# benjjneb/dada2

Measured on AMD Instinct MI355X. Metric: unique reads denoised/sec (dada() wall-clock), higher is better.
Workload: dtype int32 DP + f64 lambda/p-value

## Files before the change

dada2_amd/csrc/driver.cpp:

```cpp
#include <fcntl.h>
#include <sys/file.h>
#include <unistd.h>

#include <algorithm>
#include <atomic>
#include <chrono>
#include <condition_variable>
#include <deque>
#include <exception>
#include <mutex>
#include <cmath>
#include <cstdarg>
#include <cstdio>
#include <cstring>
#include <ctime>
#include <memory>
#include <thread>
#include <unordered_map>

#include "engine.h"
#include "hostpar.h"
#include "knobs.h"
#include "ppois.h"

// ... 45 lines not shown
  }
};

}

using namespace d2;

struct dada2hip_sample {
  int device = 0;
  hipStream_t stream = nullptr;
  hipStream_t side = nullptr;
  hipStream_t cmp = nullptr;
  SampleDev D;
  DevBuf<uint32_t> seq2, heavy, reads;
  DevBuf<uint8_t> qual, nheavy, prior;
  DevBuf<uint16_t> kord, kmult;
  DevBuf<uint32_t> kbits;
  DevBuf<int32_t> len, nwflag;
  PinBuf<uint32_t> h_seq2;
  std::vector<int32_t> h_len;
  std::vector<uint32_t> h_reads;
  std::vector<uint8_t> h_prior;
  uint64_t total_reads = 0;
  int qmax = 0;
  double ms_upload = 0;
  DevBuf<uint8_t> d_skip, d_cls, d_correct, d_moves;
  DevBuf<double> d_lambda, d_err;
  DevBuf<uint32_t> d_ham, scr_ptr, scr_t, d_qn, d_ctab, scr_adw, scr_ad;
  DevBuf<uint16_t> scr_foff;
  DevBuf<AdDesc> scr_fdesc;
  int scr_adw_waves = 0, scr_adw_band = -999;
// ... 241 lines not shown
  D2_HIP(hipMemcpyAsync(D.seq2, packed, (size_t)nraw * D.W2 * 4, hipMemcpyHostToDevice, s->stream));
  D2_HIP(hipMemcpyAsync(D.len, s->h_len.data(), (size_t)nraw * 4, hipMemcpyHostToDevice, s->stream));
  D2_HIP(hipMemcpyAsync(D.reads, s->h_reads.data(), (size_t)nraw * 4, hipMemcpyHostToDevice, s->stream));
  D2_HIP(hipMemcpyAsync(D.prior, s->h_prior.data(), (size_t)nraw, hipMemcpyHostToDevice, s->stream));
  if (lite) {
    D2_HIP(hipMemsetAsync(D.qual, 0, (size_t)nraw * D.LQ, s->stream));
    D2_HIP(hipStreamSynchronize(s->stream));
    s->qmax = 0;
    s->ms_upload = ms_since(t0);
    return;
  }
  s->kord.alloc((size_t)nraw * D.LK);
  s->heavy.alloc((size_t)nraw * std::max(D.HMAX, 1));
  D.kord = s->kord.p; D.heavy = s->heavy.p;
  if (maxlen - KMER_SIZE + 1 <= 512 && knobs().screen_bits != 0) {
    s->kbits.alloc((size_t)nraw * 32); s->kmult.alloc(nraw);
    D.kbits = s->kbits.p; D.kmult = s->kmult.p;
  } else { D.kbits = nullptr; D.kmult = nullptr; }
  launch_build_kmers(D, s->stream);

  {
    const int LQ = D.LQ;
    PinBuf<uint8_t> hq;
    hq.alloc((size_t)nraw * LQ);
    std::atomic<int> badq{0}, qmax{0};
    const int marshal_threads = active_runs(device).load() > 1 ? std::max(8, HostPool::get().nthreads() / 2) : 0;
    const size_t rows_per = std::max<size_t>(1, ((size_t)16 << 20) / (size_t)LQ);
    for (size_t r0 = 0; r0 < (size_t)nraw; r0 += rows_per) {
      const size_t nr = std::min<size_t>(rows_per, nraw - r0);
      parallel_for(nr, 512, [&](size_t lo, size_t hi) {
        int mx = 0, bad = 0;
        for (size_t r = r0 + lo; r < r0 + hi; r++) {
          const double *src = quals + r * (size_t)maxlen;
// ... 917 lines not shown
  PinBuf<Round2Out> v2_hblk;
  DevBuf<unsigned long long> v2_trace;
  int v2_trace_seq = -1;
  int v2_nbuf = 64, v2_depth = 2, v2_chain = SH_CHAIN;
  bool v2_debug = false;
  bool v3_on = false;
  int v3_depth = 1;
  int v3_grid = 1;
  int v3_bs = 1024;
  long v3_enq = 0;
  long v3_ord_seen = 0;
  DevBuf<PSync> v3_psync;
  DevBuf<int32_t> v3_lockbuf;
  int v3_lock_stride = 0;
  bool v3_pf_lowreg = false;
  bool v3_overlap = false;
  Eng2 E2P{};
  SampleDev S2{};
  DevBuf<Ctl2> v3_pfctl;
  DevBuf<PfSync> v3_pfsync;
  DevBuf<uint2> v3_pf_tab8;
  DevBuf<uint16_t> v3_pf_full, v3_pf_ord, v3_pf_foff;
  DevBuf<int32_t> v3_pf_blist, v3_pf_blistn, v3_pf_bretry, v3_pf_bretryn;
  DevBuf<uint32_t> v3_pf_ad;
  DevBuf<AdDesc> v3_pf_fdesc;
  long v3_pf_launched = 0;
  long v3_pf_seen = 0;
  long v3_pf_chains = 0;
  bool v3_pf_gate_on = true;
  hipEvent_t v3_pf_ev[4] = {nullptr, nullptr, nullptr, nullptr};
// ... 153 lines not shown

    v3_grid = tail_grid(N, s->device);
    if (K.v3_grid > 0) v3_grid = std::min(K.v3_grid, tail_grid(1 << 30, s->device));
    v3_overlap = v3_on && !v2_align_commit && v2_nbuf >= 4 && K.v3_overlap != 0 && N >= 2 && (active_runs(s->device).load() <= 1 || K.v3_overlap == 1);
    v3_bs = K.v3_block == 512 ? 512 : 1024;
    {
      const int ncu = tail_grid(1 << 30, s->device);
      if (v3_overlap && K.v3_block == 0 && K.v3_grid == 0 && v3_grid > ncu / 2) {
        v3_bs = 1024;
        v3_grid = std::max(1, std::min((N + 8191) / 8192, ncu / 2));
      }
    }
    if (v3_on) { const int cap = tail_resident_max(s->device, v3_bs); if (cap == 0 || (cap > 0 && v3_grid > cap)) v3_on = false; }
    if (!v3_on) v3_overlap = false;
    v3_pf_lowreg = K.v3_pf_lowreg >= 0 ? K.v3_pf_lowreg != 0 : (v3_overlap && v3_bs == 512);
    v3_lock_stride = 0;
    if (v3_on) {
      const long long per_group = 4096ll * v3_grid;
      v3_lock_stride = (int)(((long long)N + per_group - 1) / per_group * 4096ll);
      v3_lockbuf.alloc((size_t)v3_lock_stride * (size_t)v3_grid);
    }
    v3_pf_launched = 0; v3_pf_seen = 0; v3_pf_chains = 0;
    if (v3_overlap) {
      if (!s->cmp) D2_HIP(hipStreamCreateWithFlags(&s->cmp, hipStreamNonBlocking));
      for (auto &e : v3_pf_ev) if (!e) D2_HIP(hipEventCreateWithFlags(&e, hipEventDisableTiming));
      const size_t npad = ((size_t)N + 31) & ~(size_t)15;
      v3_pfctl.alloc(1); v3_pfsync.alloc(1); v3_pf_tab8.alloc(NKMER); v3_pf_cbits.alloc(KB_MAX * 32); v3_pf_full.alloc((size_t)KB_MAX * NKMER);
      v3_pf_ord.alloc((size_t)KB_MAX * s->D.LK + 64); v3_pf_blist.alloc((size_t)2 * KB_MAX * npad); v3_pf_blistn.alloc(2 * KB_MAX);
      v3_pf_bretry.alloc((size_t)KB_MAX * npad); v3_pf_bretryn.alloc(KB_MAX);
      D2_HIP(hipMemsetAsync(v3_pf_bretryn.p, 0, KB_MAX * 4, stq));
// ... 52 lines not shown
    st.tail_fallbacks++;
    v2_enq = v2_cons;
    v2_enqrec.assign((size_t)v2_cons, EnqRec{-1, -1, false});
    v2_next_full = 0;
    if (knobs().v2_summary) fprintf(stderr, "[v3] entry barrier failed after %ld blocks: continuing on the launch chains\n", v2_cons);
  }
  bool v3_block_ready() const { return *(volatile int32_t *)&v2_hblk.p[v2_cons % RING2].seq == (int32_t)(v2_cons + 1); }
  long v3_ended() const { return (long)*(volatile int32_t *)(v3_hflags.p + 16); }
  std::vector<EnqRec> v3_rec;
  void v3_enqueue(bool first) {
    const auto t_enq = clk::now();
    hipStream_t stq = s->stream;
    EnqRec rec{-1, -1, !first};
    if (!first) {
      rec.ev_screen = ev_begin(EV_SCREEN, profile_all, true);
      launch2_screen_multi(E2, stq);
      ev_end(rec.ev_screen);
      launch2_batch_lists(E2, stq);
      const NwBatch nb{&v2_ctl.p->nalign, v2_blistn.p, v2_blist.p, v2_ctl.p->acentre, &v2_ctl.p->abuf, E2.C.Npad, v2_bretry.p, v2_bretryn.p, v2_retrytot.p, &v2_ctl.p->fast_off};
      launch_gapless_batch(s->D, nb, ap, s->d_err.p, v2_lamB.p, v2_hamB.p, &v2_ctl.p->state, stq);
      rec.ev_nw = ev_begin(EV_NW, profile_all, true);
      launch_nw_ad(s->D, -1, nullptr, nullptr, nullptr, 0, nullptr, nullptr, ap, s->d_err.p, v2_lamB.p, v2_hamB.p, nullptr, 0, 0, nullptr, stq,
                   &v2_ctl.p->state, &nb);
      ev_end(rec.ev_nw);
    }
    const int ev = ev_begin(EV_TAIL, profile_all);
    Eng2 Ek = E2;
    if (!profile_all) Ek.ktime = nullptr;
    Ek.pf_plan = (v3_overlap && (active_runs(s->device).load() <= 1 || knobs().v3_overlap == 1)) ? 1 : 0;
    launch3_tail(Ek, v3_grid, v3_bs, first, (int)(v3_enq + 1), s->h_reads[bi[0].center], stq);
    ev_end(ev);
    v3_rec.push_back(rec);
    v3_enq++;
    st.ms_enqueue += ms_since(t_enq);
  }

  void v3_pf_enqueue(long k) {
    const auto t_enq = clk::now();
    hipStream_t st2 = s->cmp;
    Ctl2 *pc = v3_pfctl.p;
    *(volatile int32_t *)(v3_hflags.p + 40 + (k & 7)) = 0;
    launch2_pf_gate(E2P, (int)k, v3_hflags.p + 32, v3_hflags.p + 40 + (k & 7), st2);
    launch2_pf_tables(E2P, st2);
    int ev = ev_begin(EV_PF_SCREEN, profile_all, false, false, st2);
    launch2_screen_multi(E2P, st2, v3_pf_lowreg);
    ev_end(ev);
    launch2_batch_lists(E2P, st2);
    const NwBatch nb{&pc->nalign, v3_pf_blistn.p, v3_pf_blist.p, pc->acentre, &pc->abuf, E2.C.Npad, v3_pf_bretry.p, v3_pf_bretryn.p, v2_retrytot.p, &pc->fast_off};
    launch_gapless_batch(S2, nb, ap, s->d_err.p, v2_lamB.p, v2_hamB.p, &pc->state, st2);
    ev = ev_begin(EV_PF_NW, profile_all, false, false, st2);
    launch_nw_ad(S2, -1, nullptr, nullptr, nullptr, 0, nullptr, nullptr, ap, s->d_err.p, v2_lamB.p, v2_hamB.p, nullptr, 0, 0, nullptr, st2,
                 &pc->state, &nb);
    ev_end(ev);
    launch2_pf_done(E2P, st2);
    D2_HIP(hipEventRecord(v3_pf_ev[k & 3], st2));
    v3_pf_launched = std::max(v3_pf_launched, k);
    v3_pf_chains++;
    st.ms_enqueue += ms_since(t_enq);
  }
  int v3_pf_gate_result(long k) const { return (int)*(volatile int32_t *)(v3_hflags.p + 40 + (k & 7)); }
// ... 308 lines not shown
    else {
      v2_round_launches(nlev, with_compare, store, &rec, lite);
      if (with_compare) v2_plain_rounds++;
    }
    if (lite) st.lite_chains++;
    v2_enqrec.push_back(rec);
    v2_enq++;
    st.ms_enqueue += ms_since(t_enq);
  }
  void v2_round_launches(int nlev, bool with_compare, bool store, EnqRec *recp, bool lite = false) {
    hipStream_t stq = s->stream;
    EnqRec rec{-1, -1, with_compare};
    const Eng2 &E2 = lite ? this->E2L : this->E2;
    if (with_compare && !lite) {
      rec.ev_screen = ev_begin(EV_SCREEN, profile_all, true);
      launch2_screen_multi(E2, stq);
      ev_end(rec.ev_screen);
      launch2_batch_lists(E2, stq);
      const NwBatch nb{&v2_ctl.p->nalign, v2_blistn.p, v2_blist.p, v2_ctl.p->acentre, &v2_ctl.p->abuf, E2.C.Npad, v2_bretry.p, v2_bretryn.p, v2_retrytot.p, &v2_ctl.p->fast_off};
      launch_gapless_batch(s->D, nb, ap, s->d_err.p, v2_lamB.p, v2_hamB.p, &v2_ctl.p->state, stq);
      rec.ev_nw = ev_begin(EV_NW, profile_all, true);
      launch_nw_ad(s->D, -1, nullptr, nullptr, nullptr, 0, nullptr, nullptr, ap, s->d_err.p, v2_lamB.p, v2_hamB.p, nullptr, 0, 0, nullptr, stq,
                   &v2_ctl.p->state, &nb);
      ev_end(rec.ev_nw);
    }
    int ev = ev_begin(EV_SHUFFLE, profile_all && nlev > 0);
    for (int l = 0; l < nlev; l++) launch2_shuffle(E2, l, store && l == 0, stq);
    ev_end(ev);
    ev = ev_begin(EV_PVAL, profile_all);
    launch2_eval(E2, nlev, s->h_reads[bi[0].center], stq);
    ev_end(ev);
// ... 1293 lines not shown
```

dada2_amd/csrc/engine.h:

```cpp
#pragma once
#include <cstddef>
#include <cstdint>
#include <string>
#include <vector>

#include <hip/hip_runtime.h>

#include "../../include/dada2hip.h"

namespace d2 {

constexpr int KMER_SIZE = 5;
constexpr int NKMER = 1024;
constexpr int RANK_SAT = 63;
constexpr int MAX_SHUFFLE = 10;
constexpr int SEQLEN = 9999;
constexpr double TAIL_APPROX_CUTOFF = 1e-7;

enum : uint8_t { CLS_SKIP = 0, CLS_SHROUD = 1, CLS_GAPLESS = 2, CLS_NW = 3 };

struct DeviceError {
  int code;
  std::string msg;
};
// ... 7 lines not shown
  } while (0)

struct SampleDev {
  int32_t N = 0, maxlen = 0, minlen = 0;
  int32_t r_lo = 0, r_hi = 0;
  int32_t W2 = 0;
  int32_t LQ = 0;
  int32_t LK = 0;
  int32_t HMAX = 0;
  uint32_t *seq2 = nullptr;
  uint8_t *qual = nullptr;
  uint16_t *kord = nullptr;
  uint32_t *heavy = nullptr;
  uint8_t *nheavy = nullptr;
  uint32_t *kbits = nullptr;
  uint16_t *kmult = nullptr;
  int32_t *len = nullptr;
  uint32_t *reads = nullptr;
  uint8_t *prior = nullptr;
  int32_t *nw_flag = nullptr;
  uint32_t *ad_ptr = nullptr;
  int32_t ad_waves = 0;
  int32_t ad_wpw = 0;
  uint16_t *ad_foff = nullptr;
  struct AdDesc *ad_desc = nullptr;
  int32_t ad_fcap = 0, ad_fstride = 0;
};

struct AdDesc { long long dest; int32_t L2, pad; };

struct AlignParams {
// ... 312 lines not shown
};

struct PSync {
  uint32_t arrive, pad0[31];
  uint32_t gen, pad1[31];
  uint32_t fail, pad2[31];
  uint32_t top, pad3[31];
  uint32_t ngrp, pad4[31];
  uint32_t xarr[8][32], xgen[8][32], xcount[8][32], xn[8][32];
};
enum { KT_S0 = 0, KT_S0_BAR, KT_SL, KT_SL_BAR, KT_P, KT_P_BAR, KT_BIRTH, KT_PUBLISH, KT_ROUNDS, KT_LEVELS, KT_LAUNCH, KT_RELEASE,
       KT_PFWAIT , KT_PLAN , KT_SUB_LAST = 14, KT_SUB = 16, KT_N = 80 };

void launch2_store0(const Eng2 &E, const double *d_lam, const uint32_t *d_ham, const uint8_t *d_cls, const int32_t *d_round_counters,
                    hipStream_t st);
void launch2_screen_multi(const Eng2 &E, hipStream_t st, bool beside_tail = false);
void launch2_pf_gate(const Eng2 &E, int k, const int32_t *h_quit, int32_t *h_result, hipStream_t st);
void launch2_pf_tables(const Eng2 &E, hipStream_t st);
void launch2_pf_done(const Eng2 &E, hipStream_t st);
void launch2_batch_lists(const Eng2 &E, hipStream_t st);
void launch2_shuffle(const Eng2 &E, int level, bool store, hipStream_t st);
void launch2_eval(const Eng2 &E, int nlev, uint32_t init_reads, hipStream_t st);
void launch2_host_birth(const Eng2 &E, int raw, int from, hipStream_t st);
void launch2_resume(const Eng2 &E, hipStream_t st, bool keep_list = false, bool compare_done = false);
void launch2_posthoc(const Eng2 &E, const int32_t *d_cluster_of_centre, int32_t *d_out_ji, double *d_out_lam, int32_t *d_nout,
                     int cap, hipStream_t st);
int tail_grid(int N, int device);
int tail_resident_max(int device, int bs);
int tail_mirror_cap(int device, int bs);
void launch3_tail(const Eng2 &E, int grid, int bs, bool first, int ordinal, uint32_t init_reads, hipStream_t st);

// ... 13 lines not shown
```

dada2_amd/csrc/kernels.hip:

```cpp
#include <cstring>

#include "engine.h"
#include "gcn.h"
#include "knobs.h"
#include "rounds_common.h"
#include "ppois.h"

namespace d2 {

static __device__ __forceinline__ uint32_t base_at(const uint32_t *__restrict__ row, int p) {
  return (row[p >> 4] >> ((p & 15) << 1)) & 3u;
}

static __device__ __forceinline__ uint32_t homo_at(const uint32_t *__restrict__ row, int len, int p) {
  if (p < 0 || p >= len) return 0u;
  const uint32_t b = base_at(row, p);
  const int l = (p >= 1 && base_at(row, p - 1) == b) ? ((p >= 2 && base_at(row, p - 2) == b) ? 2 : 1) : 0;
  const int r = (p + 1 < len && base_at(row, p + 1) == b) ? ((p + 2 < len && base_at(row, p + 2) == b) ? 2 : 1) : 0;
  return (l + r >= 2) ? 1u : 0u;
}

__global__ __launch_bounds__(64) void k_build_kmers(SampleDev S) {
  __shared__ uint16_t tbl[NKMER * 64];
  const int lane = threadIdx.x;
// ... 16 lines not shown
      }
      for (int i = nk; i < S.LK; i++) ko[i] = 0xFFFFu;
      int nh = 0;
      if (S.HMAX > 0 || S.kbits) {
        int distinct = 0;
        for (int w = 0; w < NKMER / 32; w++) {
          uint32_t bits = 0;
          for (int b = 0; b < 32; b++) {
            const int k = 32 * w + b;
            const uint32_t c = t[k * 64];
            if (c) { bits |= 1u << b; distinct++; }
            if (S.HMAX > 0 && c > RANK_SAT) S.heavy[(size_t)r * S.HMAX + nh++] = (uint32_t)k | (c << 16);
          }
          if (S.kbits) S.kbits[(size_t)r * 32 + w] = bits;
        }
        if (S.kmult) S.kmult[r] = (uint16_t)min(max(nk, 0) - distinct, 65535);
      }
      S.nheavy[r] = (uint8_t)nh;
    }
  }
}

void launch_build_kmers(const SampleDev &S, hipStream_t st) {
  int grid = std::min((S.N + 63) / 64, 1024);
  hipLaunchKernelGGL(k_build_kmers, dim3(grid), dim3(64), 0, st, S);
}

constexpr int CTAB_SAT = 0, CTAB_CNT = 256, CTAB_ORD = 768;
static __device__ __forceinline__ void centre_table_body(const SampleDev &S, int centre, uint32_t *__restrict__ ctab, uint32_t *cnt) {
  const int tid = threadIdx.x;
  for (int k = tid; k < NKMER; k += 256) cnt[k] = 0;
// ... 2450 lines not shown
```

dada2_amd/csrc/rounds2.inc.hip:

```cpp

#ifndef D2_PUPD_INLINE
#define D2_PUPD_INLINE __forceinline__
#endif
#ifndef D2_SHUF_INLINE
#define D2_SHUF_INLINE __forceinline__
#endif
#define D2_TRACE2(KID, SUBKID, PHASE)                                                                              \
  do {                                                                                                             \
    if (E.trace && threadIdx.x == 0 && (int)blockIdx.x < TRACE_BLOCKS && E.ctl->pub_seq == E.trace_seq)           \
      E.trace[((size_t)(KID) * TRACE_BLOCKS + blockIdx.x) * 8 + (PHASE)] = gcn_clock();                            \
    D2_KSUB(SUBKID, PHASE, blockIdx.x == 0);                                                                       \
  } while (0)
#define D2_TRACE(KID, PHASE) D2_TRACE2(KID, KID, PHASE)
#define D2_TRACE_SH(LEVEL, PHASE) D2_TRACE2(1 + (LEVEL), (LEVEL) == 0 ? 1 : 2, PHASE)
#ifdef D2_TAIL_TU
static __shared__ unsigned long long s_ktime[KT_N];
#define D2_KT s_ktime
#else
#define D2_KT E.ktime
#endif
#define D2_KSUB(KID, PHASE, WHO)                                                                                   \
  do {                                                                                                             \
    if (E.ktime && threadIdx.x == 0 && (WHO)) {                                                                    \
      const unsigned long long now_ = gcn_wall_clock();                                                            \
// ... 1402 lines not shown
  build_batch_tables(E.S, E.C, nb, E.ctl->bcentre, s_cnt);
}
__global__ void k2_pf_done(Eng2 E) {
  if (threadIdx.x != 0 || E.ctl->state != 0) return;
  unsigned long long nn = 0, ng = 0;
  for (int k = 0; k < KB_MAX; k++) { nn += (unsigned long long)E.blist_n[k]; ng += (unsigned long long)E.blist_n[KB_MAX + k]; }
  E.pfsync->nnw += nn; E.pfsync->ngapless += ng;
  gcn_release_agent();
  gcn_store_agent(&E.pfsync->done, (uint32_t)E.ctl->pf_seq);
}

struct ScrIn { uint4 c0, c1; int Lr, nh; uint32_t rd; bool lk; };

template <int WAVES>
__global__ __launch_bounds__(256, WAVES) void k2_screen_multi(Eng2 E) {
  const Ctl2 *ctl = E.ctl;
  const int nb = ctl->nbatch;
  if (ctl->state != 0 || nb == 0) return;
  extern __shared__ __attribute__((aligned(16))) uint32_t s_mem[];
  const SampleDev &S = E.S;
  const Cache2 &C = E.C;
  const ScreenParams sp = E.sp;
  uint2 *tab = (uint2 *)s_mem;
  uint16_t *cord = (uint16_t *)(tab + NKMER);
  int32_t *thr = (int32_t *)(cord + (size_t)KB_MAX * S.LK);
  __shared__ int cL[KB_MAX], cC[KB_MAX];
  __shared__ uint32_t cR[KB_MAX];
  const int tid = threadIdx.x;
  for (int i = tid; i < NKMER; i += 256) tab[i] = C.tab8[i];
  {
    const int n16 = (nb * S.LK * 2 + 15) / 16;
    const uint4 *src = (const uint4 *)C.ord;
    for (int i = tid; i < n16; i += 256) ((uint4 *)cord)[i] = src[i];
  }
  for (int i = tid; i < S.maxlen + 2; i += 256) thr[i] = E.thresh[i];
  if (tid < KB_MAX) { cL[tid] = ctl->blen[tid]; cC[tid] = ctl->bcentre[tid]; cR[tid] = ctl->breads[tid]; }
  __syncthreads();
  uint16_t *bcls = C.bcls + (size_t)ctl->bbuf * C.Npad;
  const int lane = tid & 63, sub = tid & 15, g = lane >> 4;
  const int gwave = blockIdx.x * 4 + (tid >> 6), nwaves = gridDim.x * 4;
  const int nchunk = (S.maxlen - KMER_SIZE + 1 + 7) >> 3;
  const uint4 pad4 = make_uint4(0xFFFFFFFFu, 0xFFFFFFFFu, 0xFFFFFFFFu, 0xFFFFFFFFu);
  const bool heavy_on = sp.use_kmers && S.HMAX > 0;
  const int kc = sub & 7;
  const bool kvalid = sub < 8 && kc < nb;
  const int Lc = cL[kc], Cc = cC[kc];
  const uint32_t Rc = cR[kc];
  auto load = [&](int r) __attribute__((always_inline)) {
    ScrIn in;
// ... 19 lines not shown
#pragma unroll
        for (int e = 0; e < 4; e++) {
#pragma unroll
          for (int hlf = 0; hlf < 2; hlf++) {
            const uint32_t x = hlf ? (w[e] >> 16) : (w[e] & 0xFFFFu);
            const uint2 t = tab[x & 1023u];
            const uint32_t rk = x >> 10;
            const uint32_t rr = gcn_bcast_byte0(rk);
            ax += ((t.x - rr) >> 7) & 0x01010101u;
            ay += ((t.y - rr) >> 7) & 0x01010101u;
          }
        }
        w0 += ax & 0x00FF00FFu; w1 += (ax >> 8) & 0x00FF00FFu;
        w2 += ay & 0x00FF00FFu; w3 += (ay >> 8) & 0x00FF00FFu;
      }
#pragma unroll
      for (int o = 8; o >= 1; o >>= 1) {
        w0 += __shfl_xor(w0, o, 16); w1 += __shfl_xor(w1, o, 16);
        w2 += __shfl_xor(w2, o, 16); w3 += __shfl_xor(w3, o, 16);
      }
    }
    uint32_t dot = (((kc & 4) ? ((kc & 1) ? w3 : w2) : ((kc & 1) ? w1 : w0)) >> ((kc & 2) ? 16 : 0)) & 0xFFFFu;
    const bool skipped = E.greedy && (in.rd > Rc || (in.lk && r != Cc));
    if (in.nh > 0 && kvalid && !skipped) {
      for (int hh = 0; hh < in.nh; hh++) {
        const uint32_t e = S.heavy[(size_t)r * S.HMAX + hh], cr = e >> 16, cc = C.full[(size_t)kc * NKMER + (e & 1023u)];
        const uint32_t m = cr < cc ? cr : cc;
        if (m > RANK_SAT) dot += m - RANK_SAT;
      }
      dot &= 0xFFFFu;
    }
    const int d = (Lc < in.Lr ? Lc : in.Lr) - KMER_SIZE + 1;
    const bool shroud = sp.use_kmers && (int)dot < thr[d > 0 ? d : 0];
    const bool gl_ok = sp.gapless && sp.use_kmers && (sp.sse >= 1 || in.Lr == Lc);
    bool gapless = sp.band == 0;
// ... 6 lines not shown
      const uint32_t dotk = (uint32_t)__shfl((int)dot, kk, 16);
      const uint16_t *ck = cord + (size_t)kk * S.LK;
      uint32_t ord = 0;
      for (int ch = sub, j = 0; ch < nchunk; ch += 16, j++) {
        const uint4 v = j == 0 ? in.c0 : (j == 1 ? in.c1 : row[ch]);
        const uint4 ck4 = ((const uint4 *)ck)[ch];
        const uint32_t w[4] = {v.x, v.y, v.z, v.w}, cw[4] = {ck4.x, ck4.y, ck4.z, ck4.w};
        const int i0 = ch << 3;
#pragma unroll
        for (int e = 0; e < 4; e++) {
          const uint32_t t = (w[e] ^ cw[e]) & 0x03FF03FFu;
          ord += ((t & 0xFFFFu) == 0 && i0 + 2 * e < dk);
          ord += ((t >> 16) == 0 && i0 + 2 * e + 1 < dk);
        }
      }
#pragma unroll
      for (int o = 8; o >= 1; o >>= 1) ord += __shfl_xor(ord, o, 16);
      if (kc == kk && sub < 8) gapless = (ord & 0xFFFFu) == dotk;
    }
    uint32_t c = !kvalid ? 0u : (skipped ? (uint32_t)CLS_SKIP : (shroud ? (uint32_t)CLS_SHROUD : (gapless ? (uint32_t)CLS_GAPLESS : (uint32_t)CLS_NW)));
    uint32_t code = c << (2 * kc);
    code |= __shfl_xor(code, 1, 16); code |= __shfl_xor(code, 2, 16); code |= __shfl_xor(code, 4, 16);
    return code & 0xFFFFu;
  };
  const bool pre = sp.use_kmers && S.kbits != nullptr && S.kmult != nullptr && C.cbits != nullptr;
  if (!pre) {
    for (int base16 = gwave * 16; base16 < S.N; base16 += nwaves * 16) {
      const int r0 = base16 + 4 * g;
      const ScrIn i0 = load(r0), i1 = load(r0 + 1);
      unsigned long long clsacc = one(r0, i0);
      const ScrIn i2 = load(r0 + 2);
      clsacc |= (unsigned long long)one(r0 + 1, i1) << 16;
      const ScrIn i3 = load(r0 + 3);
      clsacc |= (unsigned long long)one(r0 + 2, i2) << 32;
      clsacc |= (unsigned long long)one(r0 + 3, i3) << 48;
      if (sub == 0 && r0 < S.N) *(unsigned long long *)(bcls + r0) = clsacc;
    }
    return;
  }
  constexpr int SCR_ITERS = 8, SCR_LIST = SCR_ITERS * 64;
  __shared__ int s_list[SCR_LIST];
  __shared__ int s_nlist;
  __shared__ uint2 s_cbits[KB_MAX][16];
  if (tid < KB_MAX * 16) s_cbits[tid >> 4][tid & 15] = ((const uint2 *)C.cbits)[tid];
  if (tid == 0) s_nlist = 0;
  __syncthreads();
  const int wv = tid >> 6, grp = tid >> 4;
  auto flush = [&]() __attribute__((always_inline)) {
    __syncthreads();
    const int n = s_nlist;
    for (int q = grp; q < ((n + 15) & ~15); q += 32) {
      const bool ha = q < n, hb = q + 16 < n;
      const int ra = ha ? s_list[q] : s_list[0], rb = hb ? s_list[q + 16] : s_list[0];
      const ScrIn ia = load(ra), ib = load(rb);
      const uint32_t ca = one(ra, ia), cb = one(rb, ib);
      if (sub == 0 && ha) bcls[ra] = (uint16_t)ca;
      if (sub == 0 && hb) bcls[rb] = (uint16_t)cb;
    }
    __syncthreads();
    if (tid == 0) { if (n && E.fast_ctl) atomicAdd(&E.fast_ctl[3], (unsigned long long)n); s_nlist = 0; }
    __syncthreads();
  };
  int iter = 0;
  for (long long bb = (long long)blockIdx.x * 64; bb < S.N; bb += (long long)gridDim.x * 64, iter++) {
    const int r0 = (int)bb + 16 * wv + 4 * g;
    uint2 bw[4];
    int Ls[4], kms[4];
    uint32_t rds[4];
    bool lks[4];
#pragma unroll
    for (int u = 0; u < 4; u++) {
      const int r = r0 + u;
      const bool on = r < S.N;
      bw[u] = on ? ((const uint2 *)(S.kbits + (size_t)r * 32))[sub] : make_uint2(0u, 0u);
      Ls[u] = on ? S.len[r] : 0;
      rds[u] = on ? S.reads[r] : 0u;
      lks[u] = on && E.greedy && E.P.lock[r];
      kms[u] = on ? (int)S.kmult[r] : 0;
    }
    unsigned long long clsacc = 0;
    uint32_t survs = 0;
#pragma unroll
    for (int u = 0; u < 4; u++) {
      const int r = r0 + u;
      uint32_t p[4];
#pragma unroll
      for (int kk = 0; kk < 4; kk++) {
        const uint2 c0 = s_cbits[2 * kk][sub], c1 = s_cbits[2 * kk + 1][sub];
        const uint32_t n0 = (uint32_t)__popc(bw[u].x & c0.x) + (uint32_t)__popc(bw[u].y & c0.y);
        const uint32_t n1 = (uint32_t)__popc(bw[u].x & c1.x) + (uint32_t)__popc(bw[u].y & c1.y);
        p[kk] = n0 | (n1 << 16);
      }
#pragma unroll
      for (int o = 8; o >= 1; o >>= 1) {
        p[0] += __shfl_xor(p[0], o, 16); p[1] += __shfl_xor(p[1], o, 16);
        p[2] += __shfl_xor(p[2], o, 16); p[3] += __shfl_xor(p[3], o, 16);
      }
      const uint32_t pk = (kc & 4) ? ((kc & 2) ? p[3] : p[2]) : ((kc & 2) ? p[1] : p[0]);
      const int bound = (int)((pk >> ((kc & 1) ? 16 : 0)) & 0xFFFFu) + kms[u];
      const int d = (Lc < Ls[u] ? Lc : Ls[u]) - KMER_SIZE + 1;
      const bool skipped = E.greedy && (rds[u] > Rc || (lks[u] && r != Cc));
      const bool open = kvalid && r < S.N && !skipped && !(bound < thr[d > 0 ? d : 0]);
      uint32_t code = (kvalid ? (skipped ? (uint32_t)CLS_SKIP : (uint32_t)CLS_SHROUD) : 0u) << (2 * kc);
      code |= __shfl_xor(code, 1, 16); code |= __shfl_xor(code, 2, 16); code |= __shfl_xor(code, 4, 16);
      const bool any_open = ((__ballot(open) >> (16 * g)) & 0xFFFFull) != 0ull;
      if (any_open) survs |= 1u << u;
      clsacc |= (unsigned long long)(code & 0xFFFFu) << (16 * u);
    }
    if (sub == 0 && r0 < S.N) {
      if (survs == 0) *(unsigned long long *)(bcls + r0) = clsacc;
      else {
        int at = atomicAdd(&s_nlist, __popc(survs));
#pragma unroll
        for (int u = 0; u < 4; u++) {
          if (r0 + u >= S.N) continue;
          if ((survs >> u) & 1u) s_list[at++] = r0 + u;
          else bcls[r0 + u] = (uint16_t)(clsacc >> (16 * u));
        }
      }
    }
    if ((iter % SCR_ITERS) == SCR_ITERS - 1) flush();
  }
  flush();
}

__global__ __launch_bounds__(256) void k2_posthoc(Eng2 E, const int32_t *__restrict__ cluster_of_centre, int32_t *__restrict__ out_ji,
                                                  double *__restrict__ out_lam, int32_t *__restrict__ nout, int cap) {
  const int r = blockIdx.x * blockDim.x + threadIdx.x;
  if (r >= E.S.N) return;
  const int j = cluster_of_centre[r];
  if (j < 0) return;
  if (j != 0) {
    const int k = atomicAdd(nout, 1);
    if (k < cap) { out_ji[2 * k] = j; out_ji[2 * k + 1] = 0; out_lam[k] = E.T.lam0[r]; }
  }
  const int i1 = E.T.i1[r];
  if (i1 >= 0 && i1 != j) {
    const int k = atomicAdd(nout, 1);
// ... 12 lines not shown

void launch2_store0(const Eng2 &E, const double *d_lam, const uint32_t *d_ham, const uint8_t *d_cls, const int32_t *d_round_counters,
                    hipStream_t st) {
  const int grid = std::min((E.S.N + 255) / 256, 2048);
  hipLaunchKernelGGL(k2_store0, dim3(grid), dim3(256), 0, st, E, d_lam, d_ham, d_cls, d_round_counters);
}
void launch2_batch_lists(const Eng2 &E, hipStream_t st) {
  const int grid = (E.S.N + 256 * LISTS_PER_THREAD - 1) / (256 * LISTS_PER_THREAD);
  hipLaunchKernelGGL(k2_batch_lists, dim3(grid), dim3(256), 0, st, E);
}
void launch2_pf_gate(const Eng2 &E, int k, const int32_t *h_quit, int32_t *h_result, hipStream_t st) {
  hipLaunchKernelGGL(k2_pf_gate, dim3(1), dim3(64), 0, st, E, k, h_quit, h_result);
}
void launch2_pf_tables(const Eng2 &E, hipStream_t st) { hipLaunchKernelGGL(k2_pf_tables, dim3(1), dim3(1024), 0, st, E); }
void launch2_pf_done(const Eng2 &E, hipStream_t st) { hipLaunchKernelGGL(k2_pf_done, dim3(1), dim3(64), 0, st, E); }
void launch2_screen_multi(const Eng2 &E, hipStream_t st, bool beside_tail) {
  const size_t lds = (size_t)NKMER * 8 + (size_t)KB_MAX * E.S.LK * 2 + (size_t)(E.S.maxlen + 2) * 4 + 16;
  static size_t attr_set[64] = {0};
  int dev_ = 0;
  (void)hipGetDevice(&dev_);
  if (lds > attr_set[dev_ & 63]) {
    (void)hipFuncSetAttribute((const void *)k2_screen_multi<4>, hipFuncAttributeMaxDynamicSharedMemorySize, (int)lds);
    (void)hipFuncSetAttribute((const void *)k2_screen_multi<6>, hipFuncAttributeMaxDynamicSharedMemorySize, (int)lds);
    attr_set[dev_ & 63] = lds;
  }
  const int grid = std::min((E.S.N + 63) / 64, 2048);
  if (beside_tail) hipLaunchKernelGGL(k2_screen_multi<6>, dim3(grid), dim3(256), lds, st, E);
  else hipLaunchKernelGGL(k2_screen_multi<4>, dim3(grid), dim3(256), lds, st, E);
}
void launch2_shuffle(const Eng2 &E, int level, bool store, hipStream_t st) {
  const int grid = std::min((E.S.N + 255) / 256, (int)E.grid_shuffle);
  if (store) hipLaunchKernelGGL(k2_shuffle<true>, dim3(grid), dim3(256), 0, st, E, level);
  else hipLaunchKernelGGL(k2_shuffle<false>, dim3(grid), dim3(256), 0, st, E, level);
}
void launch2_eval(const Eng2 &E, int nlev, uint32_t init_reads, hipStream_t st) {
  BudKey init{1.0, init_reads};
  const int grid = std::min((E.S.N + 255) / 256, std::min(8192, (int)E.grid_pupdate));
  hipLaunchKernelGGL(k2_pupdate, dim3(grid), dim3(256), 0, st, E, nlev, init, (BudKey *)E.partial);
  hipLaunchKernelGGL(k2_birth, dim3(1), dim3(1024), 0, st, E, nlev, init, (const BudKey *)E.partial, grid);
}
void launch2_host_birth(const Eng2 &E, int raw, int from, hipStream_t st) {
// ... 11 lines not shown
```

dada2_amd/csrc/tail.hip:

```cpp
#include <algorithm>
#include <cstdint>

#include "engine.h"
#include "gcn.h"
#include "knobs.h"
#include "ppois.h"
#include "rounds_common.h"

#define D2_TAIL_TU 1

namespace d2 {

#include "rounds2.inc.hip"
#include "rounds3.inc.hip"

}
```

Baseline: 6.753 million.

## Restructure k-mer screen kernel: packed per-read records, DPP reductions, prefetch, CU-sized grid

The k-mer screening kernel is reorganised. Each read's length, k-mer multiplicity and read count are packed into one uint2 record, so one load replaces three scattered ones. Each 8-lane half-row now processes one read with 128-bit bit-vector loads, and the next pass's data is prefetched in registers. Shuffle-based reductions are replaced with DPP row operations, and the large k-mer tables go to LDS only when some read survives the screen. The grid is now sized from the CU count, leaving room for the tail kernel when overlapped. This costs extra register pressure and more complex control flow.

```diff
diff --git a/dada2_amd/csrc/driver.cpp b/dada2_amd/csrc/driver.cpp
--- a/dada2_amd/csrc/driver.cpp
+++ b/dada2_amd/csrc/driver.cpp
@@ -83,7 +83,8 @@
   SampleDev D;
   DevBuf<uint32_t> seq2, heavy, reads;
   DevBuf<uint8_t> qual, nheavy, prior;
-  DevBuf<uint16_t> kord, kmult;
+  DevBuf<uint16_t> kord;
+  DevBuf<uint2> srec;
   DevBuf<uint32_t> kbits;
   DevBuf<int32_t> len, nwflag;
   PinBuf<uint32_t> h_seq2;
@@ -355,9 +356,9 @@
   s->heavy.alloc((size_t)nraw * std::max(D.HMAX, 1));
   D.kord = s->kord.p; D.heavy = s->heavy.p;
   if (maxlen - KMER_SIZE + 1 <= 512 && knobs().screen_bits != 0) {
-    s->kbits.alloc((size_t)nraw * 32); s->kmult.alloc(nraw);
-    D.kbits = s->kbits.p; D.kmult = s->kmult.p;
-  } else { D.kbits = nullptr; D.kmult = nullptr; }
+    s->kbits.alloc((size_t)nraw * 32); s->srec.alloc(nraw);
+    D.kbits = s->kbits.p; D.srec = s->srec.p;
+  } else { D.kbits = nullptr; D.srec = nullptr; }
   launch_build_kmers(D, s->stream);
 
   {
@@ -1305,6 +1306,7 @@
   DevBuf<int32_t> v3_lockbuf;
   int v3_lock_stride = 0;
   bool v3_pf_lowreg = false;
+  int scr_cus = 0, v3_pf_cus = 0;
   bool v3_overlap = false;
   Eng2 E2P{};
   SampleDev S2{};
@@ -1488,6 +1490,11 @@
     if (v3_on) { const int cap = tail_resident_max(s->device, v3_bs); if (cap == 0 || (cap > 0 && v3_grid > cap)) v3_on = false; }
     if (!v3_on) v3_overlap = false;
     v3_pf_lowreg = K.v3_pf_lowreg >= 0 ? K.v3_pf_lowreg != 0 : (v3_overlap && v3_bs == 512);
+    {
+      const int ncu = tail_grid(1 << 30, s->device);
+      scr_cus = ncu;
+      v3_pf_cus = (v3_overlap && v3_bs == 1024) ? std::max(1, ncu - v3_grid) : ncu;
+    }
     v3_lock_stride = 0;
     if (v3_on) {
       const long long per_group = 4096ll * v3_grid;
@@ -1570,7 +1577,7 @@
     EnqRec rec{-1, -1, !first};
     if (!first) {
       rec.ev_screen = ev_begin(EV_SCREEN, profile_all, true);
-      launch2_screen_multi(E2, stq);
+      launch2_screen_multi(E2, stq, scr_cus);
       ev_end(rec.ev_screen);
       launch2_batch_lists(E2, stq);
       const NwBatch nb{&v2_ctl.p->nalign, v2_blistn.p, v2_blist.p, v2_ctl.p->acentre, &v2_ctl.p->abuf, E2.C.Npad, v2_bretry.p, v2_bretryn.p, v2_retrytot.p, &v2_ctl.p->fast_off};
@@ -1599,7 +1606,7 @@
     launch2_pf_gate(E2P, (int)k, v3_hflags.p + 32, v3_hflags.p + 40 + (k & 7), st2);
     launch2_pf_tables(E2P, st2);
     int ev = ev_begin(EV_PF_SCREEN, profile_all, false, false, st2);
-    launch2_screen_multi(E2P, st2, v3_pf_lowreg);
+    launch2_screen_multi(E2P, st2, v3_pf_cus, v3_pf_lowreg);
     ev_end(ev);
     launch2_batch_lists(E2P, st2);
     const NwBatch nb{&pc->nalign, v3_pf_blistn.p, v3_pf_blist.p, pc->acentre, &pc->abuf, E2.C.Npad, v3_pf_bretry.p, v3_pf_bretryn.p, v2_retrytot.p, &pc->fast_off};
@@ -1938,7 +1945,7 @@
     const Eng2 &E2 = lite ? this->E2L : this->E2;
     if (with_compare && !lite) {
       rec.ev_screen = ev_begin(EV_SCREEN, profile_all, true);
-      launch2_screen_multi(E2, stq);
+      launch2_screen_multi(E2, stq, scr_cus);
       ev_end(rec.ev_screen);
       launch2_batch_lists(E2, stq);
       const NwBatch nb{&v2_ctl.p->nalign, v2_blistn.p, v2_blist.p, v2_ctl.p->acentre, &v2_ctl.p->abuf, E2.C.Npad, v2_bretry.p, v2_bretryn.p, v2_retrytot.p, &v2_ctl.p->fast_off};
diff --git a/dada2_amd/csrc/engine.h b/dada2_amd/csrc/engine.h
--- a/dada2_amd/csrc/engine.h
+++ b/dada2_amd/csrc/engine.h
@@ -45,7 +45,7 @@
   uint32_t *heavy = nullptr;
   uint8_t *nheavy = nullptr;
   uint32_t *kbits = nullptr;
-  uint16_t *kmult = nullptr;
+  uint2 *srec = nullptr;
   int32_t *len = nullptr;
   uint32_t *reads = nullptr;
   uint8_t *prior = nullptr;
@@ -388,7 +388,7 @@
 
 void launch2_store0(const Eng2 &E, const double *d_lam, const uint32_t *d_ham, const uint8_t *d_cls, const int32_t *d_round_counters,
                     hipStream_t st);
-void launch2_screen_multi(const Eng2 &E, hipStream_t st, bool beside_tail = false);
+void launch2_screen_multi(const Eng2 &E, hipStream_t st, int cus, bool beside_tail = false);
 void launch2_pf_gate(const Eng2 &E, int k, const int32_t *h_quit, int32_t *h_result, hipStream_t st);
 void launch2_pf_tables(const Eng2 &E, hipStream_t st);
 void launch2_pf_done(const Eng2 &E, hipStream_t st);
diff --git a/dada2_amd/csrc/kernels.hip b/dada2_amd/csrc/kernels.hip
--- a/dada2_amd/csrc/kernels.hip
+++ b/dada2_amd/csrc/kernels.hip
@@ -2,6 +2,7 @@
 
 #include "engine.h"
 #include "gcn.h"
+#include "lanes16.h"
 #include "knobs.h"
 #include "rounds_common.h"
 #include "ppois.h"
@@ -54,7 +55,7 @@
           }
           if (S.kbits) S.kbits[(size_t)r * 32 + w] = bits;
         }
-        if (S.kmult) S.kmult[r] = (uint16_t)min(max(nk, 0) - distinct, 65535);
+        if (S.srec) S.srec[r] = make_uint2((uint32_t)L | ((uint32_t)min(max(nk, 0) - distinct, 65535) << 16), S.reads[r]);
       }
       S.nheavy[r] = (uint8_t)nh;
     }
diff --git a/dada2_amd/csrc/lanes16.h b/dada2_amd/csrc/lanes16.h
--- /dev/null
+++ b/dada2_amd/csrc/lanes16.h
@@ -0,0 +1,41 @@
+#pragma once
+#include <hip/hip_runtime.h>
+
+namespace d2 {
+
+#if defined(__HIP_DEVICE_COMPILE__)
+template <int CTRL> static __device__ __forceinline__ uint32_t dpp_row(uint32_t x) {
+  return (uint32_t)__builtin_amdgcn_update_dpp(0, (int)x, CTRL, 0xF, 0xF, false);
+}
+constexpr int DPP_QUAD_XOR1 = 0xB1, DPP_QUAD_XOR2 = 0x4E, DPP_HALF_MIRROR = 0x141, DPP_ROR8 = 0x128, DPP_ROR4 = 0x124,
+              DPP_ROR2 = 0x122, DPP_ROR1 = 0x121;
+static __device__ __forceinline__ uint32_t row_sum16(uint32_t x) {
+  x += dpp_row<DPP_ROR8>(x); x += dpp_row<DPP_ROR4>(x); x += dpp_row<DPP_ROR2>(x); x += dpp_row<DPP_ROR1>(x);
+  return x;
+}
+static __device__ __forceinline__ uint32_t half_sum8(uint32_t x) {
+  x += dpp_row<DPP_QUAD_XOR1>(x); x += dpp_row<DPP_QUAD_XOR2>(x); x += dpp_row<DPP_HALF_MIRROR>(x);
+  return x;
+}
+static __device__ __forceinline__ uint32_t half_or8(uint32_t x) {
+  x |= dpp_row<DPP_QUAD_XOR1>(x); x |= dpp_row<DPP_QUAD_XOR2>(x); x |= dpp_row<DPP_HALF_MIRROR>(x);
+  return x;
+}
+static __device__ __forceinline__ uint32_t row_other_half(uint32_t x) { return dpp_row<DPP_ROR8>(x); }
+#else
+static __device__ __forceinline__ uint32_t row_sum16(uint32_t x) {
+  for (int o = 8; o >= 1; o >>= 1) x += __shfl_xor(x, o, 16);
+  return x;
+}
+static __device__ __forceinline__ uint32_t half_sum8(uint32_t x) {
+  for (int o = 1; o <= 4; o <<= 1) x += __shfl_xor(x, o, 16);
+  return x;
+}
+static __device__ __forceinline__ uint32_t half_or8(uint32_t x) {
+  for (int o = 1; o <= 4; o <<= 1) x |= __shfl_xor(x, o, 16);
+  return x;
+}
+static __device__ __forceinline__ uint32_t row_other_half(uint32_t x) { return __shfl_xor(x, 8, 16); }
+#endif
+
+}
diff --git a/dada2_amd/csrc/rounds2.inc.hip b/dada2_amd/csrc/rounds2.inc.hip
--- a/dada2_amd/csrc/rounds2.inc.hip
+++ b/dada2_amd/csrc/rounds2.inc.hip
@@ -1440,6 +1440,7 @@
 
 template <int WAVES>
 __global__ __launch_bounds__(256, WAVES) void k2_screen_multi(Eng2 E) {
+  constexpr int STEPS = WAVES <= 4 ? 4 : 2;
   const Ctl2 *ctl = E.ctl;
   const int nb = ctl->nbatch;
   if (ctl->state != 0 || nb == 0) return;
@@ -1453,12 +1454,17 @@
   __shared__ int cL[KB_MAX], cC[KB_MAX];
   __shared__ uint32_t cR[KB_MAX];
   const int tid = threadIdx.x;
-  for (int i = tid; i < NKMER; i += 256) tab[i] = C.tab8[i];
-  {
+  auto stage_tables = [&]() __attribute__((always_inline)) {
+    const int t = gcn_opaque_lane(tid);
+    for (int i = t; i < NKMER; i += 256) tab[i] = C.tab8[i];
     const int n16 = (nb * S.LK * 2 + 15) / 16;
     const uint4 *src = (const uint4 *)C.ord;
-    for (int i = tid; i < n16; i += 256) ((uint4 *)cord)[i] = src[i];
-  }
+    for (int i = t; i < n16; i += 256) ((uint4 *)cord)[i] = src[i];
+  };
+  const bool pre = sp.use_kmers && S.kbits != nullptr && S.srec != nullptr && C.cbits != nullptr;
+  __shared__ uint4 s_cbits[KB_MAX][8];
+  if (pre && tid < KB_MAX * 8) s_cbits[tid >> 3][tid & 7] = ((const uint4 *)C.cbits)[tid];
+  if (!pre) stage_tables();
   for (int i = tid; i < S.maxlen + 2; i += 256) thr[i] = E.thresh[i];
   if (tid < KB_MAX) { cL[tid] = ctl->blen[tid]; cC[tid] = ctl->bcentre[tid]; cR[tid] = ctl->breads[tid]; }
   __syncthreads();
@@ -1508,11 +1514,7 @@
         w0 += ax & 0x00FF00FFu; w1 += (ax >> 8) & 0x00FF00FFu;
         w2 += ay & 0x00FF00FFu; w3 += (ay >> 8) & 0x00FF00FFu;
       }
-#pragma unroll
-      for (int o = 8; o >= 1; o >>= 1) {
-        w0 += __shfl_xor(w0, o, 16); w1 += __shfl_xor(w1, o, 16);
-        w2 += __shfl_xor(w2, o, 16); w3 += __shfl_xor(w3, o, 16);
-      }
+      w0 = row_sum16(w0); w1 = row_sum16(w1); w2 = row_sum16(w2); w3 = row_sum16(w3);
     }
     uint32_t dot = (((kc & 4) ? ((kc & 1) ? w3 : w2) : ((kc & 1) ? w1 : w0)) >> ((kc & 2) ? 16 : 0)) & 0xFFFFu;
     const bool skipped = E.greedy && (in.rd > Rc || (in.lk && r != Cc));
@@ -1549,16 +1551,12 @@
           ord += ((t >> 16) == 0 && i0 + 2 * e + 1 < dk);
         }
       }
-#pragma unroll
-      for (int o = 8; o >= 1; o >>= 1) ord += __shfl_xor(ord, o, 16);
+      ord = row_sum16(ord);
       if (kc == kk && sub < 8) gapless = (ord & 0xFFFFu) == dotk;
     }
-    uint32_t c = !kvalid ? 0u : (skipped ? (uint32_t)CLS_SKIP : (shroud ? (uint32_t)CLS_SHROUD : (gapless ? (uint32_t)CLS_GAPLESS : (uint32_t)CLS_NW)));
-    uint32_t code = c << (2 * kc);
-    code |= __shfl_xor(code, 1, 16); code |= __shfl_xor(code, 2, 16); code |= __shfl_xor(code, 4, 16);
-    return code & 0xFFFFu;
+    const uint32_t c = !kvalid ? 0u : (skipped ? (uint32_t)CLS_SKIP : (shroud ? (uint32_t)CLS_SHROUD : (gapless ? (uint32_t)CLS_GAPLESS : (uint32_t)CLS_NW)));
+    return half_or8(c << (2 * kc)) & 0xFFFFu;
   };
-  const bool pre = sp.use_kmers && S.kbits != nullptr && S.kmult != nullptr && C.cbits != nullptr;
   if (!pre) {
     for (int base16 = gwave * 16; base16 < S.N; base16 += nwaves * 16) {
       const int r0 = base16 + 4 * g;
@@ -1573,90 +1571,97 @@
     }
     return;
   }
-  constexpr int SCR_ITERS = 8, SCR_LIST = SCR_ITERS * 64;
+  constexpr int SCR_LIST = 2048;
+  constexpr int PER_BLOCK = 32 * STEPS;
+  constexpr int SCR_PASSES = SCR_LIST / PER_BLOCK;
   __shared__ int s_list[SCR_LIST];
   __shared__ int s_nlist;
-  __shared__ uint2 s_cbits[KB_MAX][16];
-  if (tid < KB_MAX * 16) s_cbits[tid >> 4][tid & 15] = ((const uint2 *)C.cbits)[tid];
   if (tid == 0) s_nlist = 0;
-  __syncthreads();
   const int wv = tid >> 6, grp = tid >> 4;
+  bool staged = false;
   auto flush = [&]() __attribute__((always_inline)) {
     __syncthreads();
     const int n = s_nlist;
-    for (int q = grp; q < ((n + 15) & ~15); q += 32) {
-      const bool ha = q < n, hb = q + 16 < n;
-      const int ra = ha ? s_list[q] : s_list[0], rb = hb ? s_list[q + 16] : s_list[0];
-      const ScrIn ia = load(ra), ib = load(rb);
-      const uint32_t ca = one(ra, ia), cb = one(rb, ib);
+    if (n == 0) return;
+    if (!staged) { stage_tables(); staged = true; __syncthreads(); }
+    for (int q = gcn_opaque_lane(grp); q < ((n + 15) & ~15); q += 16) {
+      const bool ha = q < n;
+      const int ra = ha ? s_list[q] : s_list[0];
+      const uint32_t ca = one(ra, load(ra));
       if (sub == 0 && ha) bcls[ra] = (uint16_t)ca;
-      if (sub == 0 && hb) bcls[rb] = (uint16_t)cb;
     }
     __syncthreads();
-    if (tid == 0) { if (n && E.fast_ctl) atomicAdd(&E.fast_ctl[3], (unsigned long long)n); s_nlist = 0; }
+    if (tid == 0) { if (E.fast_ctl) atomicAdd(&E.fast_ctl[3], (unsigned long long)n); s_nlist = 0; }
     __syncthreads();
   };
-  int iter = 0;
-  for (long long bb = (long long)blockIdx.x * 64; bb < S.N; bb += (long long)gridDim.x * 64, iter++) {
-    const int r0 = (int)bb + 16 * wv + 4 * g;
-    uint2 bw[4];
-    int Ls[4], kms[4];
-    uint32_t rds[4];
-    bool lks[4];
-#pragma unroll
-    for (int u = 0; u < 4; u++) {
-      const int r = r0 + u;
+  const int h = sub & 7, hf = sub >> 3;
+  const bool kv1 = kc < nb;
+  struct Pass { uint4 b[STEPS]; uint2 rec[STEPS]; uint32_t lk; };
+  auto fetch = [&](long long bb) __attribute__((always_inline)) {
+    Pass f;
+    f.lk = 0;
+    const long long rb = bb + (long long)(8 * STEPS) * wv + (2 * STEPS) * g + hf;
+#pragma unroll
+    for (int s = 0; s < STEPS; s++) {
+      const long long r = rb + 2 * s;
       const bool on = r < S.N;
-      bw[u] = on ? ((const uint2 *)(S.kbits + (size_t)r * 32))[sub] : make_uint2(0u, 0u);
-      Ls[u] = on ? S.len[r] : 0;
-      rds[u] = on ? S.reads[r] : 0u;
-      lks[u] = on && E.greedy && E.P.lock[r];
-      kms[u] = on ? (int)S.kmult[r] : 0;
-    }
-    unsigned long long clsacc = 0;
-    uint32_t survs = 0;
-#pragma unroll
-    for (int u = 0; u < 4; u++) {
-      const int r = r0 + u;
-      uint32_t p[4];
-#pragma unroll
-      for (int kk = 0; kk < 4; kk++) {
-        const uint2 c0 = s_cbits[2 * kk][sub], c1 = s_cbits[2 * kk + 1][sub];
-        const uint32_t n0 = (uint32_t)__popc(bw[u].x & c0.x) + (uint32_t)__popc(bw[u].y & c0.y);
-        const uint32_t n1 = (uint32_t)__popc(bw[u].x & c1.x) + (uint32_t)__popc(bw[u].y & c1.y);
-        p[kk] = n0 | (n1 << 16);
-      }
-#pragma unroll
-      for (int o = 8; o >= 1; o >>= 1) {
-        p[0] += __shfl_xor(p[0], o, 16); p[1] += __shfl_xor(p[1], o, 16);
-        p[2] += __shfl_xor(p[2], o, 16); p[3] += __shfl_xor(p[3], o, 16);
-      }
-      const uint32_t pk = (kc & 4) ? ((kc & 2) ? p[3] : p[2]) : ((kc & 2) ? p[1] : p[0]);
-      const int bound = (int)((pk >> ((kc & 1) ? 16 : 0)) & 0xFFFFu) + kms[u];
-      const int d = (Lc < Ls[u] ? Lc : Ls[u]) - KMER_SIZE + 1;
-      const bool skipped = E.greedy && (rds[u] > Rc || (lks[u] && r != Cc));
-      const bool open = kvalid && r < S.N && !skipped && !(bound < thr[d > 0 ? d : 0]);
-      uint32_t code = (kvalid ? (skipped ? (uint32_t)CLS_SKIP : (uint32_t)CLS_SHROUD) : 0u) << (2 * kc);
-      code |= __shfl_xor(code, 1, 16); code |= __shfl_xor(code, 2, 16); code |= __shfl_xor(code, 4, 16);
-      const bool any_open = ((__ballot(open) >> (16 * g)) & 0xFFFFull) != 0ull;
-      if (any_open) survs |= 1u << u;
-      clsacc |= (unsigned long long)(code & 0xFFFFu) << (16 * u);
-    }
-    if (sub == 0 && r0 < S.N) {
-      if (survs == 0) *(unsigned long long *)(bcls + r0) = clsacc;
-      else {
-        int at = atomicAdd(&s_nlist, __popc(survs));
-#pragma unroll
-        for (int u = 0; u < 4; u++) {
-          if (r0 + u >= S.N) continue;
-          if ((survs >> u) & 1u) s_list[at++] = r0 + u;
-          else bcls[r0 + u] = (uint16_t)(clsacc >> (16 * u));
-        }
-      }
-    }
-    if ((iter % SCR_ITERS) == SCR_ITERS - 1) flush();
-  }
-  flush();
+      f.b[s] = on ? ((const uint4 *)(S.kbits + (size_t)r * 32))[h] : make_uint4(0u, 0u, 0u, 0u);
+      f.rec[s] = on ? S.srec[r] : make_uint2(0u, 0u);
+      if (on && E.greedy && E.P.lock[r]) f.lk |= 1u << s;
+    }
+    return f;
+  };
+  const long long stride = (long long)gridDim.x * PER_BLOCK;
+  for (long long seg = (long long)blockIdx.x * PER_BLOCK; seg < S.N; seg += stride * SCR_PASSES) {
+    long long bb = seg;
+    Pass cur = fetch(bb);
+    for (int pass = 0; pass < SCR_PASSES && bb < S.N; bb += stride, pass++) {
+      const Pass nxt = fetch(pass + 1 < SCR_PASSES ? bb + stride : (long long)S.N);
+      const int r0 = (int)bb + 8 * STEPS * wv + 2 * STEPS * g;
+      uint32_t cls[STEPS];
+      uint32_t survs = 0;
+#pragma unroll
+      for (int s = 0; s < STEPS; s++) {
+        const int r = r0 + 2 * s + hf;
+        const uint4 a = cur.b[s];
+        uint32_t p[4];
+#pragma unroll
+        for (int kk = 0; kk < 4; kk++) {
+          const uint4 c0 = s_cbits[2 * kk][h], c1 = s_cbits[2 * kk + 1][h];
+          const uint32_t n0 = (uint32_t)(__popc(a.x & c0.x) + __popc(a.y & c0.y) + __popc(a.z & c0.z) + __popc(a.w & c0.w));
+          const uint32_t n1 = (uint32_t)(__popc(a.x & c1.x) + __popc(a.y & c1.y) + __popc(a.z & c1.z) + __popc(a.w & c1.w));
+          p[kk] = half_sum8(n0 | (n1 << 16));
+        }
+        const uint32_t pk = (kc & 4) ? ((kc & 2) ? p[3] : p[2]) : ((kc & 2) ? p[1] : p[0]);
+        const uint2 rec = cur.rec[s];
+        const int bound = (int)((pk >> ((kc & 1) ? 16 : 0)) & 0xFFFFu) + (int)(rec.x >> 16);
+        const int Lr = (int)(rec.x & 0xFFFFu);
+        const int d = (Lc < Lr ? Lc : Lr) - KMER_SIZE + 1;
+        const bool skipped = E.greedy && (rec.y > Rc || (((cur.lk >> s) & 1u) && r != Cc));
+        const bool open = kv1 && r < S.N && !skipped && !(bound < thr[d > 0 ? d : 0]);
+        const uint32_t code = half_or8(((kv1 ? (skipped ? (uint32_t)CLS_SKIP : (uint32_t)CLS_SHROUD) : 0u) << (2 * kc)) | (open ? 0x10000u : 0u));
+        const uint32_t code1 = row_other_half(code);
+        cls[s] = (code & 0xFFFFu) | (code1 << 16);
+        survs |= ((code >> 16) | ((code1 >> 16) << 1)) << (2 * s);
+      }
+      if (sub == 0 && r0 < S.N) {
+        if (survs == 0) {
+          if constexpr (STEPS == 4) *(uint4 *)(bcls + r0) = make_uint4(cls[0], cls[1], cls[2], cls[3]);
+          else *(uint2 *)(bcls + r0) = make_uint2(cls[0], cls[1]);
+        } else {
+          int at = atomicAdd(&s_nlist, __popc(survs));
+#pragma unroll
+          for (int j = 0; j < 2 * STEPS; j++) {
+            if (r0 + j >= S.N) continue;
+            if ((survs >> j) & 1u) s_list[at++] = r0 + j;
+            else bcls[r0 + j] = (uint16_t)(cls[j >> 1] >> (16 * (j & 1)));
+          }
+        }
+      }
+      cur = nxt;
+    }
+    flush();
+  }
 }
 
 __global__ __launch_bounds__(256) void k2_posthoc(Eng2 E, const int32_t *__restrict__ cluster_of_centre, int32_t *__restrict__ out_ji,
@@ -1699,9 +1704,10 @@
 }
 void launch2_pf_tables(const Eng2 &E, hipStream_t st) { hipLaunchKernelGGL(k2_pf_tables, dim3(1), dim3(1024), 0, st, E); }
 void launch2_pf_done(const Eng2 &E, hipStream_t st) { hipLaunchKernelGGL(k2_pf_done, dim3(1), dim3(64), 0, st, E); }
-void launch2_screen_multi(const Eng2 &E, hipStream_t st, bool beside_tail) {
+void launch2_screen_multi(const Eng2 &E, hipStream_t st, int cus, bool beside_tail) {
   const size_t lds = (size_t)NKMER * 8 + (size_t)KB_MAX * E.S.LK * 2 + (size_t)(E.S.maxlen + 2) * 4 + 16;
   static size_t attr_set[64] = {0};
+  static int ncu_of[64] = {0};
   int dev_ = 0;
   (void)hipGetDevice(&dev_);
   if (lds > attr_set[dev_ & 63]) {
@@ -1709,7 +1715,15 @@
     (void)hipFuncSetAttribute((const void *)k2_screen_multi<6>, hipFuncAttributeMaxDynamicSharedMemorySize, (int)lds);
     attr_set[dev_ & 63] = lds;
   }
-  const int grid = std::min((E.S.N + 63) / 64, 2048);
+  if (cus <= 0) {
+    if (ncu_of[dev_ & 63] <= 0) {
+      hipDeviceProp_t prop;
+      ncu_of[dev_ & 63] = (hipGetDeviceProperties(&prop, dev_) == hipSuccess && prop.multiProcessorCount > 0) ? prop.multiProcessorCount : 64;
+    }
+    cus = ncu_of[dev_ & 63];
+  }
+  const int per_cu = beside_tail ? 3 : 4;
+  const int grid = std::max(1, std::min((E.S.N + 63) / 64, std::max(cus * per_cu, (E.S.N + 2047) / 2048)));
   if (beside_tail) hipLaunchKernelGGL(k2_screen_multi<6>, dim3(grid), dim3(256), lds, st, E);
   else hipLaunchKernelGGL(k2_screen_multi<4>, dim3(grid), dim3(256), lds, st, E);
 }
diff --git a/dada2_amd/csrc/tail.hip b/dada2_amd/csrc/tail.hip
--- a/dada2_amd/csrc/tail.hip
+++ b/dada2_amd/csrc/tail.hip
@@ -3,6 +3,7 @@
 
 #include "engine.h"
 #include "gcn.h"
+#include "lanes16.h"
 #include "knobs.h"
 #include "ppois.h"
 #include "rounds_common.h"
```

Result: faster. 6.938 million, median of 6 (+2.7%).
